# LingmaFuture/PRCV2025REID

Hardware: AMD Instinct MI355X
Metric: multimodal instances/sec (PxK, 5-modality) at 1/2/4/8 GPU; eval queries/sec (higher is better)
Workload: dtype bf16; 1 GPU; P=16,K=4 per GPU, vis/nir/sk/cp 224x224 + text (T<=77), CLIP ViT-B/16 + text tower random-init, MER-LoRA r=8, masks all-on, 400 ids, SDM+CE, fwd+bwd+grad sanitise/clip+AdamW (reference default trainable set); P=16, K=4, global_batch=64, lora_rank=8, accum_steps=1, parallelism=dp1

## Files before the change

### include/reid_hip.h

```cpp
#ifndef REID_HIP_H
#define REID_HIP_H

#include <stdint.h>

#ifdef __cplusplus
extern "C" {
#endif

typedef enum {
    REID_OK = 0,
    REID_ERR_ARG = -1,
    REID_ERR_LAUNCH = -2,
    REID_ERR_DEVICE = -3
} reid_status;

typedef enum { REID_BF16 = 0, REID_F32 = 1, REID_F16 = 2 } reid_dtype;

typedef enum {
    REID_ACT_NONE = 0,
    REID_ACT_GELU_ERF = 1,
    REID_ACT_QUICK_GELU = 2,
    REID_ACT_RELU = 3,
    REID_ACT_DGELU_ERF = 4,
    REID_ACT_DQUICK_GELU = 5,
// ... 41 lines not shown
int reid_add_layernorm_fwd(const float* x, int32_t ldx, const void* y_bf16, int32_t y_dtype, int32_t ldy, const float* row_scale, int32_t rows_per_img,
                           float* x_out, int32_t ldxo, const float* gamma, const float* beta, void* h_bf16, int32_t ldh,
                           float* mean, float* rstd, int32_t rows, int32_t cols, float eps, void* stream);
int reid_layernorm_bwd(const void* dy, int32_t dy_dtype, int32_t lddy, const float* x, int32_t ldx,
                       const int32_t* row_index, const float* gamma, const float* mean, const float* rstd,
                       const void* dres, void* dx, int32_t dx_dtype, void* dx_bf16, int32_t lddx,
                       float* dgamma, float* dbeta, int32_t rows, int32_t cols,
                       const float* bf16_row_scale, int32_t rows_per_img, int32_t* overflow, void* stream);

int reid_patch_im2col(const float* images, void* patches, int32_t n_img, int32_t H, int32_t W,
                      int32_t patch, int32_t cin, void* stream);
int reid_cls_rows(const float* cls, const float* pos0, float* x, int32_t ldx, int32_t n_img,
                  int32_t tokens, int32_t cols, void* stream);

int reid_attn_fwd(const void* qkv, int32_t ld, const uint8_t* key_mask, void* out, int32_t ldo, float* lse,
                  int32_t n_seq, int32_t S, int32_t heads, int32_t causal, int32_t q_tiles, void* stream);
int reid_attn_bwd(const void* qkv, int32_t ld, const uint8_t* key_mask, const void* out, const void* dout,
                  int32_t ldo, const float* lse, void* dqkv, int32_t lddqkv, float* delta_ws,
                  int32_t n_seq, int32_t S, int32_t heads, int32_t causal, int32_t q_tiles, void* stream);

int reid_cast_f32_bf16(const float* src, void* dst, int64_t n, void* stream);
int reid_cast_bf16_f32(const void* src, float* dst, int64_t n, void* stream);
int reid_pack_bf16_table(const float* src, void* dst_bf16, const int64_t* table, int32_t n_entries, void* stream);
int reid_lora_bwd_fused(const void* dY, int32_t lddy, const void* T, int32_t ldt, const void* BT, int32_t ldbt, void* U, int32_t ldu,
                        float* dB, int32_t lddb, const int32_t* img_mod, int32_t rows_per_img, int32_t mask_r, int32_t M, int32_t N,
                        int32_t Rp, float scale, float* u_partial, int32_t u_mode, void* stream);
int reid_lora_da_fused(const void* X, int32_t ldx, const void* U, int32_t ldu, float* dA, int32_t ldda, const int32_t* img_mod,
                       int32_t rows_per_img, int32_t mask_r, int32_t M, int32_t K, int32_t Rp, int32_t n_groups, void* stream);

int reid_merge_lora_table(const int64_t* table, int32_t n_entries, int32_t max_tiles, const float* arena, void* weff,
                          int32_t Rp, int32_t r, int32_t nmod, float scaling, void* stream);
int reid_gather_rows_f32(const float* src, int32_t lds, const int32_t* index, float* dst, int32_t ldd,
                         int32_t rows, int32_t cols, void* stream);
int reid_embed_tokens(const float* tok, const float* pos, const int64_t* ids, float* out, int32_t B, int32_t T, int32_t D,
                      int32_t vocab, void* stream);
int reid_scatter_add_rows_f32(const float* src, int32_t lds, const int32_t* index, float* out, int32_t ldo,
                              int32_t rows, int32_t cols, int32_t out_rows, void* stream);

int reid_bnneck_stats(const float* x, int32_t ldx, int32_t rows, int32_t D, float* sum, float* sqsum, void* stream);
int reid_bnneck_fwd(const float* x, int32_t ldx, const float* gamma, const float* beta, float* running_mean,
                    float* running_var, const float* sum, const float* sqsum, float count, int32_t training,
                    float* y, void* y_bf16, int32_t ldy, float* mean, float* invstd, float* rnorm,
                    int32_t rows, int32_t D, float eps, float momentum, float scale, void* stream);
int reid_bnneck_bwd_p1(const float* dy, int32_t lddy, const float* x, int32_t ldx, const float* gamma,
                       const float* beta, const float* mean, const float* invstd, const float* rnorm,
                       float* dz, float* sum_dz, float* sum_dz_xhat, int32_t rows, int32_t D, float scale,
                       void* stream);
int reid_bnneck_bwd_p2(const float* dz, const float* x, int32_t ldx, const float* gamma, const float* mean,
                       const float* invstd, const float* sum_dz, const float* sum_dz_xhat, float count,
                       int32_t training, float* dx, int32_t lddx, int32_t rows, int32_t D, void* stream);

// ... 67 lines not shown
```

### prcv2025reid_amd/_lib.py

```python
import ctypes as C
import os

import torch

_HERE = os.path.dirname(os.path.abspath(__file__))
LIB_PATHS = {'bf16': os.path.join(_HERE, 'csrc', 'libreid_hip.so'), 'f16': os.path.join(_HERE, 'csrc', 'libreid_hip_f16.so')}
if os.environ.get('REID_LIB_BF16'):
    LIB_PATHS['bf16'] = os.environ['REID_LIB_BF16']
LIB_PATH = LIB_PATHS['bf16']
T16_DTYPES = {'bf16': torch.bfloat16, 'f16': torch.float16}
_flavor = os.environ.get('REID_T16', 'bf16')


def set_flavor(name: str):
    global _flavor
    if name not in LIB_PATHS:
        raise ValueError(f'unknown 16-bit flavor {name!r}')
    _flavor = name


def flavor() -> str:
    return _flavor


# ... 23 lines not shown
                ('b_group_stride', C.c_int64)]


_P, _I, _I64, _F, _S = C.c_void_p, C.c_int32, C.c_int64, C.c_float, C.c_char_p
_GEMM = C.POINTER(GemmArgs)
SIGNATURES = {
    'reid_last_error': (_S, []),
    'reid_version': (_I, []),
    'reid_flavor': (_I, []),
    'reid_check_device': (_I, [_I]),
    'reid_set_knob': (_I, [_S, _I]),
    'reid_mer_gemm': (_I, [_GEMM, _P]),
    'reid_gemm_tn': (_I, [_P, _P, _P, _I, _I, _I, _I, _I, _I, _F, _F, _P]),
    'reid_layernorm_fwd': (_I, [_P, _I, _P, _P, _P, _P, _P, _I, _P, _P, _I, _I, _F, _P]),
    'reid_add_layernorm_fwd': (_I, [_P, _I, _P, _I, _I, _P, _I, _P, _I, _P, _P, _P, _I, _P, _P, _I, _I, _F, _P]),
    'reid_layernorm_bwd': (_I, [_P, _I, _I, _P, _I, _P, _P, _P, _P, _P, _P, _I, _P, _I, _P, _P, _I, _I, _P, _I, _P, _P]),
    'reid_patch_im2col': (_I, [_P, _P, _I, _I, _I, _I, _I, _P]),
    'reid_cls_rows': (_I, [_P, _P, _P, _I, _I, _I, _I, _P]),
    'reid_attn_fwd': (_I, [_P, _I, _P, _P, _I, _P, _I, _I, _I, _I, _I, _P]),
    'reid_attn_bwd': (_I, [_P, _I, _P, _P, _P, _I, _P, _P, _I, _P, _I, _I, _I, _I, _I, _P]),
    'reid_cast_f32_bf16': (_I, [_P, _P, _I64, _P]),
    'reid_cast_bf16_f32': (_I, [_P, _P, _I64, _P]),
    'reid_pack_bf16_table': (_I, [_P, _P, _P, _I, _P]),
    'reid_lora_bwd_fused': (_I, [_P, _I, _P, _I, _P, _I, _P, _I, _P, _I, _P, _I, _I, _I, _I, _I, _F, _P, _I, _P]),
    'reid_lora_da_fused': (_I, [_P, _I, _P, _I, _P, _I, _P, _I, _I, _I, _I, _I, _I, _P]),
    'reid_merge_lora_table': (_I, [_P, _I, _I, _P, _P, _I, _I, _I, _F, _P]),
    'reid_gather_rows_f32': (_I, [_P, _I, _P, _P, _I, _I, _I, _P]),
    'reid_embed_tokens': (_I, [_P, _P, _P, _P, _I, _I, _I, _I, _P]),
    'reid_scatter_add_rows_f32': (_I, [_P, _I, _P, _P, _I, _I, _I, _I, _P]),
    'reid_bnneck_stats': (_I, [_P, _I, _I, _I, _P, _P, _P]),
    'reid_bnneck_fwd': (_I, [_P, _I, _P, _P, _P, _P, _P, _P, _F, _I, _P, _P, _I, _P, _P, _P, _I, _I, _F, _F, _F, _P]),
    'reid_bnneck_bwd_p1': (_I, [_P, _I, _P, _I, _P, _P, _P, _P, _P, _P, _P, _P, _I, _I, _F, _P]),
    'reid_bnneck_bwd_p2': (_I, [_P, _P, _I, _P, _P, _P, _P, _P, _F, _I, _P, _I, _I, _I, _P]),
    'reid_ce_ls_fwd': (_I, [_P, _I, _P, _P, _I, _I, _F, _P, _P, _P]),
    'reid_ce_ls_bwd': (_I, [_P, _I, _P, _P, _I, _I, _F, _P, _P, _I, _P]),
    'reid_sdm_fwd': (_I, [_P, _I, _P, _I, _P, _P, _P, _P, _I, _I, _I, _I, _F, _P, _P, _P]),
    'reid_sdm_bwd': (_I, [_P, _I, _P, _I, _P, _P, _P, _P, _I, _I, _I, _I, _F, _P, _P, _P, _I, _P, _I, _P]),
    'reid_sdm_ws_floats': (_I64, [_I, _I, _I, _I]),
    'reid_topk_ws_bytes': (_I64, [_I, _I, _I]),
    'reid_topk_scan_ok': (_I, [_I, _I, _I, _I]),
    'reid_cosine_topk': (_I, [_P, _P, _P, _P, _I, _I, _I, _I, _P, _P, _P, _P, _P, _P]),
    'reid_cosine_topk_exact': (_I, [_P, _P, _I, _I, _I, _I, _P, _P, _P, _P, _P, _P]),
    'reid_cosine_topk_exact_slots': (_I, [_P, _P, _I, _I, _I, _I, _P, _P, _I, _P, _P, _P, _P, _P]),
    'reid_topk_stream_ok': (_I, [_I, _I, _I, _I]),
    'reid_topk_stream_ws_bytes': (_I64, [_I]),
    'reid_cosine_topk_stream': (_I, [_P, _P, _I, _I, _I, _I, _P, _P, _P, _P, _P, _P]),
    'reid_sgemm': (_I, [_P, _P, _P, _I, _I, _I, _I64, _I64, _I64, _I64, _I, _F, _F, _P, _I, _P]),
    'reid_eltwise_f32': (_I, [_I, _P, _P, _P, _I64, _F, _P]),
# ... 91 lines not shown
```

### prcv2025reid_amd/csrc/lora.hip

```cpp
#include "common.h"
#include <type_traits>

namespace {

constexpr int MT = 64;

__global__ __launch_bounds__(256) void merge_lora_kernel(const int64_t* __restrict__ table, const float* __restrict__ arena,
                                                         bf16_t* __restrict__ weff, int Rp, int r, int nmod, float s) {
    REID_T16_ENTER();
    const int64_t* e = table + (size_t)blockIdx.y * 8;
    const int N = (int)e[5], K = (int)e[6], G = (int)e[7];
    const int tiles_k = K / MT;
    if ((int)blockIdx.x >= (N / MT) * tiles_k) return;
    const float* __restrict__ W = (const float*)e[0];
    const float* __restrict__ A = arena + e[1];
    const float* __restrict__ B = arena + e[2];
    bf16_t* dst = weff + e[3];
    bf16_t* dstT = e[4] >= 0 ? weff + e[4] : nullptr;
    const int n0 = ((int)blockIdx.x / tiles_k) * MT, k0 = ((int)blockIdx.x % tiles_k) * MT;
    const int g = n0 / (N / G);
    const int R = nmod * r;
    __shared__ __attribute__((aligned(16))) float sW[MT][MT + 4];
    __shared__ __attribute__((aligned(16))) float sA[MT][MT + 4];
    __shared__ __attribute__((aligned(16))) float sBt[MT][MT + 4];
// ... 67 lines not shown
}

namespace fused {
constexpr int N = 768, RP = 32, R = 32;
constexpr int TP = RP * 2 + 32;
template <int NW> struct Geo {
    static constexpr int CPW = N / NW, MT = CPW / 16, KS = CPW / 32, CH = CPW / 8, XL = R * CH / 64;
    static constexpr int XP = CPW * 2 + 32;
    static constexpr int WAVE_LDS = R * XP + R * TP;
    static constexpr int LDS_BYTES = NW * WAVE_LDS + NW * R * RP * 4;
};

typedef __attribute__((ext_vector_type(4))) short s4;
typedef __attribute__((address_space(3))) s4* lds_s4_ptr;
typedef float f32x2v __attribute__((ext_vector_type(2)));

struct Params {
    const bf16_t* dY; const bf16_t* T; const bf16_t* BT; bf16_t* U; float* dB;
    const int32_t* img_mod;
    int lddy, ldt, ldbt, ldu, lddb, rows_per_img, mask_r, M, slab_rows;
    float scale;
    float* Up;
    int u_mode;
};

__device__ __forceinline__ bf16x8 tr_frag(const char* img, int pitch, int k0, int col0, int lane) {
    const int l16 = lane & 15, fq = lane >> 4;
    const int q = l16 >> 2, pp = l16 & 3;
    const char* a0 = img + (k0 + 4 * fq + q) * pitch + (col0 + 4 * pp) * 2;
    const s4 lo = __builtin_amdgcn_ds_read_tr16_b64_v4i16((lds_s4_ptr)(a0));
    const s4 hi = __builtin_amdgcn_ds_read_tr16_b64_v4i16((lds_s4_ptr)(a0 + 16 * pitch));
    return bf16x8{lo[0], lo[1], lo[2], lo[3], hi[0], hi[1], hi[2], hi[3]};
}

template <int NW>
__global__ __launch_bounds__(NW * 64, 2) void lora_bwd_fused_kernel(const Params p) {
    REID_T16_ENTER();
    using G = Geo<NW>;
    constexpr int CPW = G::CPW, MT = G::MT, KS = G::KS, CH = G::CH, XL = G::XL, XP = G::XP, WAVE_LDS = G::WAVE_LDS;
    extern __shared__ __attribute__((aligned(16))) char smem[];
    const int tid = threadIdx.x, lane = tid & 63;
    const int w = __builtin_amdgcn_readfirstlane(tid >> 6);
    const int l16 = lane & 15, fq = lane >> 4;
    char* xs = smem + w * WAVE_LDS;
    char* ts = xs + R * XP;
    float* ured = (float*)(smem + NW * WAVE_LDS);
// ... 86 lines not shown
    gload(0);
    for (int t = 0; t < steps; ++t) step(t);
#pragma unroll
    for (int i = 0; i < MT; ++i)
#pragma unroll
        for (int j = 0; j < 2; ++j)
#pragma unroll
            for (int e = 0; e < 4; ++e)
                atomicAdd(p.dB + (size_t)(col0 + i * 16 + 4 * fq + e) * p.lddb + j * 16 + l16, acc[i][j][e]);
}
}

namespace image {
constexpr int N = fused::N, RP = fused::RP, R = 32;
constexpr int ROW_BYTES = N * 2;
constexpr int IMG_BYTES = R * ROW_BYTES;
constexpr int T_BYTES = R * RP * 2;
constexpr int BUF_BYTES = IMG_BYTES + T_BYTES;
constexpr int NBUF = 3;
constexpr int USTAGE_BYTES = R * RP * 2;
constexpr int LDS_BYTES = NBUF * BUF_BYTES + USTAGE_BYTES;
typedef const __attribute__((address_space(1))) void* gptr_t;
typedef __attribute__((address_space(3))) void* lptr_t;
using fused::s4; using fused::lds_s4_ptr; using fused::Params;

typedef __attribute__((address_space(3))) char* lds_cptr;
__device__ __forceinline__ uint32_t lds_addr(const char* ptr) { return (uint32_t)(uintptr_t)(lds_cptr)(char*)ptr; }
__device__ __forceinline__ void dma16(const void* src, uint32_t lds_base) {
    const uint32_t m0v = __builtin_amdgcn_readfirstlane(lds_base);
    asm volatile("s_mov_b32 m0, %1\n\ts_nop 0\n\tglobal_load_lds_dwordx4 %0, off" ::"v"(src), "s"(m0v) : "memory");
}

__device__ __forceinline__ bf16x8 tr_frag_swz(const char* img, int col0, int lane) {
    const int l16 = lane & 15, fq = lane >> 4;
    const int q = l16 >> 2, pp = l16 & 3;
    const int col = col0 + 4 * pp;
    const int r0 = 4 * fq + q, r1 = r0 + 16;
    const char* a0 = img + r0 * ROW_BYTES + (((col >> 3) ^ (r0 & 15)) << 4) + (col & 7) * 2;
    const char* a1 = img + r1 * ROW_BYTES + (((col >> 3) ^ (r1 & 15)) << 4) + (col & 7) * 2;
    const s4 lo = __builtin_amdgcn_ds_read_tr16_b64_v4i16((lds_s4_ptr)a0);
    const s4 hi = __builtin_amdgcn_ds_read_tr16_b64_v4i16((lds_s4_ptr)a1);
    return bf16x8{lo[0], lo[1], lo[2], lo[3], hi[0], hi[1], hi[2], hi[3]};
}

__global__ __launch_bounds__(256) void u_finish_kernel(const float* __restrict__ Up, bf16_t* __restrict__ U, int ldu, const int32_t* __restrict__ img_mod,
                                                       int rows_per_img, int mask_r, float scale, int M) {
    REID_T16_ENTER();
// ... 132 lines not shown
                }
            }
            const int cbase = (w - 2) * 128;
#pragma unroll
            for (int i = 0; i < 8; ++i) acc[i] = mfma16(tr_frag_swz(xs, cbase + i * 16, lane), tf, acc[i]);
        }
        const int nb = buf == 0 ? NBUF - 1 : buf - 1;
        if (t + 2 < steps) issue(t + 2, nb);
        buf = buf + 1 == NBUF ? 0 : buf + 1;
    }
    if (w < 2) flush_pending();
    __syncthreads();
    float* fl = (float*)smem;
    if (w >= 2) {
        const int cbase = (w - 2) * 128;
#pragma unroll
        for (int i = 0; i < 8; ++i)
#pragma unroll
            for (int e = 0; e < 4; ++e) fl[(cbase + i * 16 + 4 * fq + e) * 16 + l16] = acc[i][e];
    }
    __syncthreads();
    {
        const int rr = p.mask_r, total = N * rr;
        for (int idx = tid; idx < total; idx += 512) {
            const int col = idx / rr, j = idx - col * rr;
            atomicAdd(p.dB + (size_t)col * p.lddb + mu * rr + j, fl[col * 16 + c_lo + j]);
        }
    }
}

struct DaParams {
    const bf16_t* X; const bf16_t* U; float* dA;
    const int32_t* img_mod;
    int ldx, ldu, ldda, rows_per_img, mask_r, M, Rp;
};
template <int G>
__global__ __launch_bounds__(512, 2) void lora_da_image_kernel(const DaParams p) {
    REID_T16_ENTER();
    constexpr int UB = 4096;
    constexpr int BUF = IMG_BYTES + UB;
    extern __shared__ __attribute__((aligned(16))) char smem[];
    const int tid = threadIdx.x, lane = tid & 63;
    const int w = __builtin_amdgcn_readfirstlane(tid >> 6);
    const int l16 = lane & 15, fq = lane >> 4;
    const int img = blockIdx.x, cblk = blockIdx.y;
    const int rbeg = img * p.rows_per_img;
    const int rend = min(p.M, rbeg + p.rows_per_img);
    if (rbeg >= rend) return;
    const int mu = p.img_mod[img];
    const int w0 = (mu * p.mask_r) & ~15;
    const int c_lo = mu * p.mask_r - w0, c_hi = c_lo + p.mask_r;
    const int steps = (rend - rbeg + R - 1) / R;
    const bf16_t* Xb = p.X + (size_t)cblk * N;
    const uint32_t smem_a = lds_addr(smem);
    auto issue = [&](int t, int buf) {
        const uint32_t base = smem_a + buf * BUF;
        const int r0 = rbeg + t * R;
// ... 33 lines not shown
        const char* xs = smem + buf * BUF;
        const char* us = xs + IMG_BYTES;
        const int nvalid = rend - (rbeg + t * R);
        bf16x8 uf[G];
#pragma unroll
        for (int g = 0; g < G; ++g) {
            uf[g] = fused::tr_frag(us + g * 1024, 32, 0, 0, lane);
            if (nvalid < R) {
#pragma unroll
                for (int j = 0; j < 8; ++j)
                    if (16 * (j >> 2) + 4 * fq + (j & 3) >= nvalid) uf[g][j] = 0;
            }
        }
#pragma unroll
        for (int i = 0; i < 6; ++i) {
            const bf16x8 xf = tr_frag_swz(xs, w * 96 + i * 16, lane);
#pragma unroll
            for (int g = 0; g < G; ++g) acc[g][i] = mfma16(uf[g], xf, acc[g][i]);
        }
        const int nb = buf == 0 ? NBUF - 1 : buf - 1;
        if (t + 2 < steps) issue(t + 2, nb);
        buf = buf + 1 == NBUF ? 0 : buf + 1;
    }
#pragma unroll
    for (int e = 0; e < 4; ++e) {
        const int c = 4 * fq + e;
        if (c < c_lo || c >= c_hi) continue;
#pragma unroll
        for (int g = 0; g < G; ++g)
#pragma unroll
            for (int i = 0; i < 6; ++i)
                atomicAdd(p.dA + (size_t)(g * p.Rp + w0 + c) * p.ldda + (size_t)cblk * N + w * 96 + i * 16 + l16, acc[g][i][e]);
    }
}
}

}

extern "C" int reid_lora_bwd_fused(const void* dY, int32_t lddy, const void* T, int32_t ldt, const void* BT, int32_t ldbt, void* U,
                                   int32_t ldu, float* dB, int32_t lddb, const int32_t* img_mod, int32_t rows_per_img, int32_t mask_r,
                                   int32_t M, int32_t N, int32_t Rp, float scale, float* u_partial, int32_t u_mode, void* stream) {
    REID_CHECK_ARG(u_mode >= 0 && u_mode <= 3 && (u_mode == 0 || u_partial), "reid_lora_bwd_fused: u_mode=%d needs u_partial", u_mode);
    REID_CHECK_ARG(dY && T && BT && U && dB && img_mod, "reid_lora_bwd_fused: null pointer");
    REID_CHECK_ARG(N == fused::N && Rp == fused::RP, "reid_lora_bwd_fused: N=%d Rp=%d (this kernel is built for N = 768, Rp = 32)", N, Rp);
    REID_CHECK_ARG(M > 0 && rows_per_img > 0 && mask_r > 0 && mask_r <= Rp, "reid_lora_bwd_fused: M=%d rows_per_img=%d mask_r=%d", M, rows_per_img, mask_r);
    REID_CHECK_ARG(lddy % 8 == 0 && ldt % 8 == 0 && ldbt % 8 == 0 && ldu % 2 == 0 && lddy >= N && ldt >= Rp && ldbt >= N && ldu >= Rp && lddb >= Rp,
                   "reid_lora_bwd_fused: leading dimensions");
    REID_CHECK_ARG(((uintptr_t)dY | (uintptr_t)T | (uintptr_t)BT) % 16 == 0 && (uintptr_t)U % 4 == 0, "reid_lora_bwd_fused: operand alignment");
    fused::Params p{(const bf16_t*)dY, (const bf16_t*)T, (const bf16_t*)BT, (bf16_t*)U, dB, img_mod, lddy, ldt, ldbt, ldu, lddb, rows_per_img,
                    mask_r, M, 0, scale, u_partial, u_mode};
    if (reid_knob(KNOB_LORA_IMPL) != 1 && rows_per_img >= image::R && mask_r <= 16 && 16 % mask_r == 0) {
        REID_MAX_LDS((image::lora_bwd_image_kernel), image::LDS_BYTES);
        const int n_img = (M + rows_per_img - 1) / rows_per_img;
        hipLaunchKernelGGL(image::lora_bwd_image_kernel, dim3(n_img), dim3(512), image::LDS_BYTES, (hipStream_t)stream, p);
        REID_CHECK_LAUNCH("reid_lora_bwd_fused(image)");
        if (u_mode == 1) {
            hipLaunchKernelGGL(image::u_finish_kernel, dim3((M * 16 + 255) / 256), dim3(256), 0, (hipStream_t)stream, (const float*)u_partial, (bf16_t*)U,
                               ldu, img_mod, rows_per_img, mask_r, scale, M);
            REID_CHECK_LAUNCH("reid_lora_bwd_fused(finish)");
        }
        return REID_OK;
    }
    int slabs = 64;
    p.slab_rows = ((M + slabs - 1) / slabs + fused::R - 1) / fused::R * fused::R;
    slabs = (M + p.slab_rows - 1) / p.slab_rows;
    REID_MAX_LDS((fused::lora_bwd_fused_kernel<8>), fused::Geo<8>::LDS_BYTES);
    hipLaunchKernelGGL(fused::lora_bwd_fused_kernel<8>, dim3(slabs), dim3(512), fused::Geo<8>::LDS_BYTES, (hipStream_t)stream, p);
    REID_CHECK_LAUNCH("reid_lora_bwd_fused");
    return REID_OK;
}

extern "C" int reid_lora_da_fused(const void* X, int32_t ldx, const void* U, int32_t ldu, float* dA, int32_t ldda, const int32_t* img_mod,
                                  int32_t rows_per_img, int32_t mask_r, int32_t M, int32_t K, int32_t Rp, int32_t n_groups, void* stream) {
    REID_CHECK_ARG(X && U && dA && img_mod, "reid_lora_da_fused: null pointer");
    REID_CHECK_ARG(M > 0 && K > 0 && K % 768 == 0 && Rp == 32 && (n_groups == 1 || n_groups == 3), "reid_lora_da_fused: M=%d K=%d Rp=%d groups=%d (K a multiple of 768, Rp = 32, 1 or 3 groups)", M, K, Rp, n_groups);
    REID_CHECK_ARG(rows_per_img >= image::R && mask_r > 0 && mask_r <= 16 && 16 % mask_r == 0, "reid_lora_da_fused: rows_per_img=%d (>= 32) mask_r=%d (a divisor of 16)", rows_per_img, mask_r);
    REID_CHECK_ARG(ldx % 8 == 0 && ldu % 8 == 0 && ldx >= K && ldu >= n_groups * Rp && ldda >= K, "reid_lora_da_fused: leading dimensions");
    REID_CHECK_ARG(((uintptr_t)X | (uintptr_t)U) % 16 == 0, "reid_lora_da_fused: operand alignment");
    image::DaParams p{(const bf16_t*)X, (const bf16_t*)U, dA, img_mod, ldx, ldu, ldda, rows_per_img, mask_r, M, Rp};
    const int n_img = (M + rows_per_img - 1) / rows_per_img;
    constexpr int LDS = image::NBUF * (image::IMG_BYTES + 4096);
    if (n_groups == 1) {
        REID_MAX_LDS((image::lora_da_image_kernel<1>), LDS);
        hipLaunchKernelGGL(image::lora_da_image_kernel<1>, dim3(n_img, K / 768), dim3(512), LDS, (hipStream_t)stream, p);
    } else {
        REID_MAX_LDS((image::lora_da_image_kernel<3>), LDS);
        hipLaunchKernelGGL(image::lora_da_image_kernel<3>, dim3(n_img, K / 768), dim3(512), LDS, (hipStream_t)stream, p);
    }
    REID_CHECK_LAUNCH("reid_lora_da_fused");
    return REID_OK;
}

extern "C" int reid_merge_lora_table(const int64_t* table, int32_t n_entries, int32_t max_tiles, const float* arena, void* weff,
                                     int32_t Rp, int32_t r, int32_t nmod, float scaling, void* stream) {
    REID_CHECK_ARG(table && arena && weff, "reid_merge_lora_table: null pointer");
    REID_CHECK_ARG(n_entries > 0 && n_entries <= 65535 && max_tiles > 0, "reid_merge_lora_table: n_entries=%d max_tiles=%d", n_entries, max_tiles);
    REID_CHECK_ARG(r > 0 && nmod > 0 && r <= MT && nmod * r <= Rp, "reid_merge_lora_table: r = %d must be <= %d and nmod*r = %d <= Rp = %d", r, MT, nmod * r, Rp);
    hipLaunchKernelGGL(merge_lora_kernel, dim3(max_tiles, n_entries), dim3(256), 0, (hipStream_t)stream, table, arena, (bf16_t*)weff, Rp, r, nmod,
                       scaling);
    REID_CHECK_LAUNCH("reid_merge_lora_table");
    return REID_OK;
}
```

### prcv2025reid_amd/engine.py

```python
from collections import OrderedDict
from typing import Dict, List, Optional, Tuple

import os

import torch

from . import _lib, ops

LIN = ('qkv', 'out', 'fc1', 'fc2')


def round_up(a, b):
    return (a + b - 1) // b * b


class LoraLayout:

    def __init__(self, arch):
        self.vmods = [m for m in arch['modalities'] if m != 'text']
        self.nmod = len(self.vmods)
        self.r = arch['lora_rank']
        self.Rp = round_up(self.nmod * self.r, 32)
        self.d = arch['vision_hidden_dim']; self.ff = arch['vision_mlp_dim']
        self.L = arch['vision_layers']
# ... 411 lines not shown
        dgf, dbf = ln_grads(ce + 'vision_ln_final')
        ops.layernorm_bwd(dcls, st['x_final'], P[ce + 'vision_ln_final.weight'], st['mf'], st['rf'], dx_c, dx_bf16=dxb_c,
                          bf16_row_scale=st['layers'][-1]['sm'], rows_per_img=1, dgamma=dgf, dbeta=dbf, overflow=ovf)
        U2 = torch.empty(M, Rp, **b16); U1 = torch.empty(M, Rp, **b16); Uo = torch.empty(M, Rp, **b16)
        Uq = torch.empty(M, 3 * Rp, **b16)
        du2 = [torch.empty(M, ff, **b16) for _ in range(2)]
        dqkv2 = [torch.empty(M, 3 * d, **b16) for _ in range(2)]
        dxmb2 = [torch.empty(M, d, **b16) for _ in range(2)]
        dxb2 = [dxb, torch.empty(M, d, **b16)]
        dh = torch.empty(M, d, **b16); do = torch.empty(M, d, **b16)
        delta = torch.empty(n_img, heads, S, **f32)
        dxm = torch.empty(M, d, **gx)
        weT = lambda l, nm: lay.weff(self._weff, l, nm, transposed=True)
        rg_full, rg_cls = st['rg_full'], st['rg_cls']
        main = torch.cuda.current_stream(dev)
        side = self._side_stream() if self.overlap_tn else None
        side_done = {}
        L = a['vision_layers']
        u_part = torch.empty(M, Rp, **f32)
        cls_tmp = dict(U2=torch.empty(n_img, Rp, **b16), U1=torch.empty(n_img, Rp, **b16), Uo=torch.empty(n_img, Rp, **b16),
                       du=torch.empty(n_img, ff, **b16), dh=torch.empty(n_img, d, **b16), do=torch.empty(n_img, d, **b16),
                       dxm=torch.empty(n_img, d, **gx), dxmb=torch.empty(n_img, d, **b16))

        def lora_grads(l, calls):
            def run():
                for dY, BT, U, kw, tns in calls:
                    same = tns[0][0].data_ptr() == dY.data_ptr() and tns[0][0].shape == dY.shape and tns[0][0].stride() == dY.stride()
                    if same and ops.lora_bwd_fused_ok(dY.shape[1], tns[0][1].shape[1]):
                        ops.lora_bwd_fused(dY, tns[0][1], BT, U, tns[0][2], kw['img_mod'], kw['rows_per_img'], kw['mask_r'], kw['alpha'],
                                           u_partial=u_part[:dY.shape[0]] if dY.shape[1] > 768 else None)
                        rest = tns[1:]
                    else:
                        ops.gemm(dY, BT, U, **kw)
                        rest = tns
                    for xx, yy, out in rest:
                        ng = xx.shape[1] // Rp
                        if xx.shape[1] == ng * Rp and out.shape[0] == ng * Rp and \
                                ops.lora_da_fused_ok(yy.shape[1], Rp, kw['rows_per_img'], kw['mask_r'], ng):
                            ops.lora_da_fused(yy, xx, out, kw['img_mod'], kw['rows_per_img'], kw['mask_r'], n_groups=ng)
                        else:
                            ops.gemm_tn(xx, yy, out, beta=1.0)
            if side is None:
                run()
                return
            ev = torch.cuda.Event(); ev.record(main); side.wait_event(ev)
            with torch.cuda.stream(side):
                run()

        def layer_done(l):
            if side is not None:
                ev = torch.cuda.Event(); ev.record(side); side_done[l] = ev

        def wait_side(l):
            ev = side_done.pop(l, None)
            if ev is not None:
                main.wait_event(ev)

        for l in reversed(range(L)):
            s = st['layers'][l]
            lp = f'{ce}vision_layers.{l}.'
            b = l & 1
            c = bool(s.get('cls'))
            if c:
                Mr, rg = n_img, rg_cls
                mkr = dict(img_mod=st['img_mod'], mask_r=r, mask_period=Rp, rows_per_img=1, alpha=self.scaling)
                gy, gyb = dx_c, dxb_c
                U2r, U1r, Uor, dur, dhr, dor, dxmr, dxmbr = (cls_tmp[k_] for k_ in ('U2', 'U1', 'Uo', 'du', 'dh', 'do', 'dxm', 'dxmb'))
                rpi = 1
            else:
                Mr, mkr, gy, gyb, rg = M, mk, dx, dxb2[b], rg_full
                U2r, U1r, Uor, dur, dhr, dor, dxmr, dxmbr, rpi = U2, U1, Uo, du2[b], dh, do, dxm, dxmb2[b], S
            dqkv = dqkv2[b]
            lora_grads(l, [(gyb, pk(l, 'fc2', 'BT'), U2r, mkr, [(gyb, s['T2'], gB(l, 'fc2')), (U2r, s['g'], gA(l, 'fc2'))])])
            ops.gemm(gyb, weT(l, 'fc2'), dur, act='mul_aux', aux=s['u'], row_groups=rg)
# ... 260 lines not shown
```

### prcv2025reid_amd/ops.py

```python
import ctypes as C
from typing import Optional

import torch

from . import _lib as L
from ._lib import BF16, F32, GemmArgs, check, lib, ptr, stream_ptr

ACT = {'none': L.ACT_NONE, 'gelu': L.ACT_GELU, 'quick_gelu': L.ACT_QUICK_GELU, 'relu': L.ACT_RELU,
       'dgelu': L.ACT_DGELU, 'dquick_gelu': L.ACT_DQUICK_GELU, 'drelu': L.ACT_DRELU,
       'mul_aux': L.ACT_MUL_AUX, 'gelu_dsave': L.ACT_GELU_DSAVE}


_gemm_profile = None
def gemm_profile_begin():
    global _gemm_profile
    _gemm_profile = []


def gemm_profile_end():
    global _gemm_profile
    p, _gemm_profile = _gemm_profile, None
    return p


# ... 116 lines not shown
    n, _, H, W = images.shape
    check(lib().reid_patch_im2col(ptr(images), ptr(patches), n, H, W, patch, cin, stream_ptr()))


def cls_rows(cls, pos0, x, n_img, tokens):
    check(lib().reid_cls_rows(ptr(cls), ptr(pos0), ptr(x), x.stride(0), n_img, tokens, x.shape[1], stream_ptr()))


def attn_fwd(qkv, out, lse, n_seq, S, heads, causal=False, key_mask=None, q_tiles=0):
    check(lib().reid_attn_fwd(ptr(qkv), qkv.stride(0), ptr(key_mask), ptr(out), out.stride(0), ptr(lse), n_seq, S, heads,
                              int(causal), int(q_tiles), stream_ptr()))


def attn_bwd(qkv, out, dout, lse, dqkv, delta_ws, n_seq, S, heads, causal=False, key_mask=None, q_tiles=0):
    check(lib().reid_attn_bwd(ptr(qkv), qkv.stride(0), ptr(key_mask), ptr(out), ptr(dout), out.stride(0), ptr(lse),
                              ptr(dqkv), dqkv.stride(0), ptr(delta_ws), n_seq, S, heads, int(causal), int(q_tiles), stream_ptr()))


def cast_f32_bf16(src, dst):
    check(lib().reid_cast_f32_bf16(ptr(src), ptr(dst), src.numel(), stream_ptr()))
    return dst


def lora_bwd_fused(dY, T, BT, U, dB, img_mod, rows_per_img, mask_r, scale, u_partial=None):
    N = dY.shape[1]
    nb = N // 768
    if nb > 1 and u_partial is None:
        raise ValueError('lora_bwd_fused: a cotangent wider than 768 columns needs u_partial')
    for q in range(nb):
        mode = 0 if nb == 1 else ((1 if q > 0 else 0) | (2 if q + 1 < nb else 0))
        dYq, BTq, dBq = dY[:, q * 768:(q + 1) * 768], BT[:, q * 768:(q + 1) * 768], dB[q * 768:(q + 1) * 768]
        check(lib().reid_lora_bwd_fused(ptr(dYq), dYq.stride(0), ptr(T), T.stride(0), ptr(BTq), BTq.stride(0), ptr(U), U.stride(0),
                                        ptr(dBq), dBq.stride(0), ptr(img_mod), rows_per_img, mask_r, dY.shape[0], 768, T.shape[1],
                                        scale, ptr(u_partial), mode, stream_ptr()))


def lora_da_fused(X, U, dA, img_mod, rows_per_img, mask_r, n_groups=1):
    check(lib().reid_lora_da_fused(ptr(X), X.stride(0), ptr(U), U.stride(0), ptr(dA), dA.stride(0), ptr(img_mod), rows_per_img, mask_r,
                                   X.shape[0], X.shape[1], U.shape[1] // n_groups, n_groups, stream_ptr()))


def lora_da_fused_ok(K, Rp, rows_per_img, mask_r, n_groups):
    return K % 768 == 0 and Rp == 32 and rows_per_img >= 32 and mask_r <= 16 and 16 % mask_r == 0 and n_groups in (1, 3)


def lora_bwd_fused_ok(N, Rp):
    return N % 768 == 0 and N // 768 in (1, 2, 3, 4) and Rp == 32


def merge_lora_table(table, n_entries, max_tiles, arena, weff, Rp, r, nmod, scaling):
    check(lib().reid_merge_lora_table(ptr(table), n_entries, max_tiles, ptr(arena), ptr(weff), Rp, r, nmod, scaling, stream_ptr()))


def to_bf16(src: torch.Tensor) -> torch.Tensor:
    src = src.contiguous()
    dst = torch.empty(src.shape, dtype=L.t16(), device=src.device)
    if src.numel():
        cast_f32_bf16(src, dst)
    return dst


def pack_bf16_table(src_arena, dst_arena, table, n_entries):
# ... 149 lines not shown
```

Baseline: 2131 instances/s.

## Replace LoRA gradient atomics with per-image partials and batched deferred reduction

The fused LoRA backward kernels (dB and dA) used to atomically add per-image contributions into the gradient buffers. They now write per-image partials into a per-stream workspace. A new batched reduce kernel sums those partials by modality mask, and it runs once per layer for up to 16 entries. This targets atomic contention and nondeterminism, at the cost of extra workspace memory, extra memory traffic, and an additional reduce launch per layer.

Result: no change. 2129 instances/s, median of 3 (-0.1%).

```diff
diff --git a/include/reid_hip.h b/include/reid_hip.h
--- a/include/reid_hip.h
+++ b/include/reid_hip.h
@@ -87,11 +87,14 @@
 int reid_cast_f32_bf16(const float* src, void* dst, int64_t n, void* stream);
 int reid_cast_bf16_f32(const void* src, float* dst, int64_t n, void* stream);
 int reid_pack_bf16_table(const float* src, void* dst_bf16, const int64_t* table, int32_t n_entries, void* stream);
-int reid_lora_bwd_fused(const void* dY, int32_t lddy, const void* T, int32_t ldt, const void* BT, int32_t ldbt, void* U, int32_t ldu,
-                        float* dB, int32_t lddb, const int32_t* img_mod, int32_t rows_per_img, int32_t mask_r, int32_t M, int32_t N,
-                        int32_t Rp, float scale, float* u_partial, int32_t u_mode, void* stream);
-int reid_lora_da_fused(const void* X, int32_t ldx, const void* U, int32_t ldu, float* dA, int32_t ldda, const int32_t* img_mod,
-                       int32_t rows_per_img, int32_t mask_r, int32_t M, int32_t K, int32_t Rp, int32_t n_groups, void* stream);
+int reid_lora_bwd_fused_ws(const void* dY, int32_t lddy, const void* T, int32_t ldt, const void* BT, int32_t ldbt, void* U, int32_t ldu,
+                           float* dB, int32_t lddb, const int32_t* img_mod, int32_t rows_per_img, int32_t mask_r, int32_t M, int32_t N,
+                           int32_t Rp, float scale, float* u_partial, int32_t u_mode, float* workspace, int64_t workspace_bytes,
+                           int32_t defer, void* stream);
+int reid_lora_da_fused_ws(const void* X, int32_t ldx, const void* U, int32_t ldu, float* dA, int32_t ldda, const int32_t* img_mod,
+                          int32_t rows_per_img, int32_t mask_r, int32_t M, int32_t K, int32_t Rp, int32_t n_groups, float* workspace,
+                          int64_t workspace_bytes, int32_t defer, void* stream);
+int reid_lora_reduce_partials(const int64_t* entries, int32_t n_entries, void* stream);
 
 int reid_merge_lora_table(const int64_t* table, int32_t n_entries, int32_t max_tiles, const float* arena, void* weff,
                           int32_t Rp, int32_t r, int32_t nmod, float scaling, void* stream);
diff --git a/prcv2025reid_amd/_lib.py b/prcv2025reid_amd/_lib.py
--- a/prcv2025reid_amd/_lib.py
+++ b/prcv2025reid_amd/_lib.py
@@ -69,8 +69,9 @@
     'reid_cast_f32_bf16': (_I, [_P, _P, _I64, _P]),
     'reid_cast_bf16_f32': (_I, [_P, _P, _I64, _P]),
     'reid_pack_bf16_table': (_I, [_P, _P, _P, _I, _P]),
-    'reid_lora_bwd_fused': (_I, [_P, _I, _P, _I, _P, _I, _P, _I, _P, _I, _P, _I, _I, _I, _I, _I, _F, _P, _I, _P]),
-    'reid_lora_da_fused': (_I, [_P, _I, _P, _I, _P, _I, _P, _I, _I, _I, _I, _I, _I, _P]),
+    'reid_lora_bwd_fused_ws': (_I, [_P, _I, _P, _I, _P, _I, _P, _I, _P, _I, _P, _I, _I, _I, _I, _I, _F, _P, _I, _P, _I64, _I, _P]),
+    'reid_lora_da_fused_ws': (_I, [_P, _I, _P, _I, _P, _I, _P, _I, _I, _I, _I, _I, _I, _P, _I64, _I, _P]),
+    'reid_lora_reduce_partials': (_I, [_P, _I, _P]),
     'reid_merge_lora_table': (_I, [_P, _I, _I, _P, _P, _I, _I, _I, _F, _P]),
     'reid_gather_rows_f32': (_I, [_P, _I, _P, _P, _I, _I, _I, _P]),
     'reid_embed_tokens': (_I, [_P, _P, _P, _P, _I, _I, _I, _I, _P]),
diff --git a/prcv2025reid_amd/csrc/lora.hip b/prcv2025reid_amd/csrc/lora.hip
--- a/prcv2025reid_amd/csrc/lora.hip
+++ b/prcv2025reid_amd/csrc/lora.hip
@@ -113,6 +113,7 @@
     float scale;
     float* Up;
     int u_mode;
+    float* dBp;
 };
 
 __device__ __forceinline__ bf16x8 tr_frag(const char* img, int pitch, int k0, int col0, int lane) {
@@ -245,7 +246,7 @@
 constexpr int LDS_BYTES = NBUF * BUF_BYTES + USTAGE_BYTES;
 typedef const __attribute__((address_space(1))) void* gptr_t;
 typedef __attribute__((address_space(3))) void* lptr_t;
-using fused::s4; using fused::lds_s4_ptr; using fused::Params;
+using fused::s4; using fused::lds_s4_ptr; using fused::Params; using fused::f32x2v;
 
 typedef __attribute__((address_space(3))) char* lds_cptr;
 __device__ __forceinline__ uint32_t lds_addr(const char* ptr) { return (uint32_t)(uintptr_t)(lds_cptr)(char*)ptr; }
@@ -424,17 +425,18 @@
     __syncthreads();
     {
         const int rr = p.mask_r, total = N * rr;
+        float* part = p.dBp + (size_t)img * total;
         for (int idx = tid; idx < total; idx += 512) {
             const int col = idx / rr, j = idx - col * rr;
-            atomicAdd(p.dB + (size_t)col * p.lddb + mu * rr + j, fl[col * 16 + c_lo + j]);
+            part[idx] = fl[col * 16 + c_lo + j];
         }
     }
 }
 
 struct DaParams {
-    const bf16_t* X; const bf16_t* U; float* dA;
+    const bf16_t* X; const bf16_t* U; float* dAp;
     const int32_t* img_mod;
-    int ldx, ldu, ldda, rows_per_img, mask_r, M, Rp;
+    int ldx, ldu, rows_per_img, mask_r, M, Rp;
 };
 template <int G>
 __global__ __launch_bounds__(512, 2) void lora_da_image_kernel(const DaParams p) {
@@ -514,6 +516,8 @@
         if (t + 2 < steps) issue(t + 2, nb);
         buf = buf + 1 == NBUF ? 0 : buf + 1;
     }
+    const int rr = p.mask_r;
+    float* part = p.dAp + ((size_t)img * gridDim.y + cblk) * G * rr * N;
 #pragma unroll
     for (int e = 0; e < 4; ++e) {
         const int c = 4 * fq + e;
@@ -521,35 +525,135 @@
 #pragma unroll
         for (int g = 0; g < G; ++g)
 #pragma unroll
-            for (int i = 0; i < 6; ++i)
-                atomicAdd(p.dA + (size_t)(g * p.Rp + w0 + c) * p.ldda + (size_t)cblk * N + w * 96 + i * 16 + l16, acc[g][i][e]);
-    }
-}
-}
-
-}
-
-extern "C" int reid_lora_bwd_fused(const void* dY, int32_t lddy, const void* T, int32_t ldt, const void* BT, int32_t ldbt, void* U,
-                                   int32_t ldu, float* dB, int32_t lddb, const int32_t* img_mod, int32_t rows_per_img, int32_t mask_r,
-                                   int32_t M, int32_t N, int32_t Rp, float scale, float* u_partial, int32_t u_mode, void* stream) {
-    REID_CHECK_ARG(u_mode >= 0 && u_mode <= 3 && (u_mode == 0 || u_partial), "reid_lora_bwd_fused: u_mode=%d needs u_partial", u_mode);
-    REID_CHECK_ARG(dY && T && BT && U && dB && img_mod, "reid_lora_bwd_fused: null pointer");
-    REID_CHECK_ARG(N == fused::N && Rp == fused::RP, "reid_lora_bwd_fused: N=%d Rp=%d (this kernel is built for N = 768, Rp = 32)", N, Rp);
-    REID_CHECK_ARG(M > 0 && rows_per_img > 0 && mask_r > 0 && mask_r <= Rp, "reid_lora_bwd_fused: M=%d rows_per_img=%d mask_r=%d", M, rows_per_img, mask_r);
+            for (int i = 0; i < 6; ++i) part[(size_t)(g * rr + c - c_lo) * N + w * 96 + i * 16 + l16] = acc[g][i][e];
+    }
+}
+
+enum { RED_DB = 0, RED_DA = 1 };
+struct RedEntry {
+    const float* part; float* dst; const int32_t* img_mod;
+    int n_img, Q, r, ld, G, mode;
+};
+constexpr int RED_MAX = 16, RED_Q = 128, RED_U = 16;
+struct RedBatch { RedEntry e[RED_MAX]; };
+
+__device__ __forceinline__ size_t red_dst(const RedEntry& p, int q, int mu) {
+    if (p.mode == RED_DB) {
+        const int col = q / p.r, j = q - col * p.r;
+        return (size_t)col * p.ld + mu * p.r + j;
+    }
+    const int k = q % N, a = q / N;
+    const int j = a % p.r, cg = a / p.r, g = cg % p.G, cblk = cg / p.G;
+    return (size_t)(g * RP + mu * p.r + j) * p.ld + (size_t)cblk * N + k;
+}
+
+template <int NMU, int NW>
+__global__ __launch_bounds__(NW * 64) void lora_partial_reduce_kernel(const RedBatch b) {
+    REID_T16_ENTER();
+    __shared__ __attribute__((aligned(16))) float red[NW][RED_Q];
+    __shared__ unsigned presw[NW];
+    const RedEntry p = b.e[blockIdx.y];
+    if ((int)blockIdx.x * RED_Q >= p.Q) return;
+    const int tid = threadIdx.x, lane = tid & 63;
+    const int w = __builtin_amdgcn_readfirstlane(tid >> 6);
+    const int q0 = blockIdx.x * RED_Q + 2 * lane;
+    float dv[NMU];
+    if (tid < RED_Q) {
+#pragma unroll
+        for (int k = 0; k < NMU; ++k) dv[k] = k * p.r < RP ? p.dst[red_dst(p, blockIdx.x * RED_Q + tid, k)] : 0.f;
+    }
+    const int i0 = (int)((int64_t)p.n_img * w / NW), i1 = (int)((int64_t)p.n_img * (w + 1) / NW);
+    f32x2v acc[NMU];
+#pragma unroll
+    for (int k = 0; k < NMU; ++k) acc[k] = f32x2v{0.f, 0.f};
+    unsigned pres = 0u;
+    for (int i = i0; i < i1; i += RED_U) {
+        const int mv = lane < RED_U && i + lane < i1 ? p.img_mod[i + lane] : -1;
+        f32x2v v[RED_U];
+#pragma unroll
+        for (int u = 0; u < RED_U; ++u) {
+            const int ii = min(i + u, i1 - 1);
+            v[u] = *(const f32x2v*)(p.part + (size_t)ii * p.Q + q0);
+        }
+#pragma unroll
+        for (int u = 0; u < RED_U; ++u) {
+            const int mu = __builtin_amdgcn_readlane(mv, u);
+            if (mu >= 0 && mu < NMU) pres |= 1u << mu;
+#pragma unroll
+            for (int k = 0; k < NMU; ++k)
+                if (mu == k) acc[k] += v[u];
+        }
+    }
+    if (lane == 0) presw[w] = pres;
+    __syncthreads();
+    unsigned all = 0u;
+#pragma unroll
+    for (int ww = 0; ww < NW; ++ww) all |= presw[ww];
+#pragma unroll
+    for (int k = 0; k < NMU; ++k) {
+        if (!((all >> k) & 1u)) continue;
+        *(f32x2v*)&red[w][2 * lane] = acc[k];
+        __syncthreads();
+        if (tid < RED_Q) {
+            float s = red[0][tid];
+#pragma unroll
+            for (int ww = 1; ww < NW; ++ww) s += red[ww][tid];
+            p.dst[red_dst(p, blockIdx.x * RED_Q + tid, k)] = dv[k] + s;
+        }
+        __syncthreads();
+    }
+}
+
+int launch_partial_reduce(const RedBatch& b, int n, hipStream_t stream) {
+    int rmin = 16, qmax = 0;
+    for (int i = 0; i < n; ++i) { rmin = min(rmin, b.e[i].r); qmax = max(qmax, b.e[i].Q); }
+    const dim3 grid(qmax / RED_Q, n);
+    const int nmu = RP / rmin;
+    if (nmu <= 4) hipLaunchKernelGGL((lora_partial_reduce_kernel<4, 16>), grid, dim3(16 * 64), 0, stream, b);
+    else if (nmu <= 8) hipLaunchKernelGGL((lora_partial_reduce_kernel<8, 16>), grid, dim3(16 * 64), 0, stream, b);
+    else if (nmu <= 16) hipLaunchKernelGGL((lora_partial_reduce_kernel<16, 8>), grid, dim3(8 * 64), 0, stream, b);
+    else hipLaunchKernelGGL((lora_partial_reduce_kernel<32, 8>), grid, dim3(8 * 64), 0, stream, b);
+    return 0;
+}
+}
+
+}
+
+extern "C" int reid_lora_bwd_fused_ws(const void* dY, int32_t lddy, const void* T, int32_t ldt, const void* BT, int32_t ldbt, void* U,
+                                      int32_t ldu, float* dB, int32_t lddb, const int32_t* img_mod, int32_t rows_per_img, int32_t mask_r,
+                                      int32_t M, int32_t N, int32_t Rp, float scale, float* u_partial, int32_t u_mode, float* workspace,
+                                      int64_t workspace_bytes, int32_t defer, void* stream) {
+    REID_CHECK_ARG(u_mode >= 0 && u_mode <= 3 && (u_mode == 0 || u_partial), "reid_lora_bwd_fused_ws: u_mode=%d needs u_partial", u_mode);
+    REID_CHECK_ARG(dY && T && BT && U && dB && img_mod, "reid_lora_bwd_fused_ws: null pointer");
+    REID_CHECK_ARG(N == fused::N && Rp == fused::RP, "reid_lora_bwd_fused_ws: N=%d Rp=%d (this kernel is built for N = 768, Rp = 32)", N, Rp);
+    REID_CHECK_ARG(M > 0 && rows_per_img > 0 && mask_r > 0 && mask_r <= Rp, "reid_lora_bwd_fused_ws: M=%d rows_per_img=%d mask_r=%d", M, rows_per_img, mask_r);
     REID_CHECK_ARG(lddy % 8 == 0 && ldt % 8 == 0 && ldbt % 8 == 0 && ldu % 2 == 0 && lddy >= N && ldt >= Rp && ldbt >= N && ldu >= Rp && lddb >= Rp,
-                   "reid_lora_bwd_fused: leading dimensions");
-    REID_CHECK_ARG(((uintptr_t)dY | (uintptr_t)T | (uintptr_t)BT) % 16 == 0 && (uintptr_t)U % 4 == 0, "reid_lora_bwd_fused: operand alignment");
+                   "reid_lora_bwd_fused_ws: leading dimensions");
+    REID_CHECK_ARG(((uintptr_t)dY | (uintptr_t)T | (uintptr_t)BT) % 16 == 0 && (uintptr_t)U % 4 == 0, "reid_lora_bwd_fused_ws: operand alignment");
+    const bool image_shape = rows_per_img >= image::R && mask_r <= 16 && 16 % mask_r == 0;
+    const int n_img = (M + rows_per_img - 1) / rows_per_img;
+    const int64_t need = (int64_t)n_img * N * mask_r * (int64_t)sizeof(float);
+    REID_CHECK_ARG(!defer || image_shape, "reid_lora_bwd_fused_ws: defer needs the one-image-per-workgroup shape (rows_per_img >= 32, mask_r a divisor of 16)");
     fused::Params p{(const bf16_t*)dY, (const bf16_t*)T, (const bf16_t*)BT, (bf16_t*)U, dB, img_mod, lddy, ldt, ldbt, ldu, lddb, rows_per_img,
-                    mask_r, M, 0, scale, u_partial, u_mode};
-    if (reid_knob(KNOB_LORA_IMPL) != 1 && rows_per_img >= image::R && mask_r <= 16 && 16 % mask_r == 0) {
+                    mask_r, M, 0, scale, u_partial, u_mode, workspace};
+    if (image_shape) {
+        REID_CHECK_ARG(workspace && workspace_bytes >= need && (uintptr_t)workspace % 16 == 0,
+                       "reid_lora_bwd_fused_ws: workspace of %lld bytes (16-byte aligned) needed, %lld given", (long long)need, (long long)workspace_bytes);
+    }
+    if (image_shape && reid_knob(KNOB_LORA_IMPL) != 1) {
         REID_MAX_LDS((image::lora_bwd_image_kernel), image::LDS_BYTES);
-        const int n_img = (M + rows_per_img - 1) / rows_per_img;
         hipLaunchKernelGGL(image::lora_bwd_image_kernel, dim3(n_img), dim3(512), image::LDS_BYTES, (hipStream_t)stream, p);
-        REID_CHECK_LAUNCH("reid_lora_bwd_fused(image)");
+        REID_CHECK_LAUNCH("reid_lora_bwd_fused_ws(image)");
+        if (!defer) {
+            image::RedBatch b{};
+            b.e[0] = image::RedEntry{workspace, dB, img_mod, n_img, N * mask_r, mask_r, lddb, 1, image::RED_DB};
+            image::launch_partial_reduce(b, 1, (hipStream_t)stream);
+            REID_CHECK_LAUNCH("reid_lora_bwd_fused_ws(reduce)");
+        }
         if (u_mode == 1) {
             hipLaunchKernelGGL(image::u_finish_kernel, dim3((M * 16 + 255) / 256), dim3(256), 0, (hipStream_t)stream, (const float*)u_partial, (bf16_t*)U,
                                ldu, img_mod, rows_per_img, mask_r, scale, M);
-            REID_CHECK_LAUNCH("reid_lora_bwd_fused(finish)");
+            REID_CHECK_LAUNCH("reid_lora_bwd_fused_ws(finish)");
         }
         return REID_OK;
     }
@@ -558,19 +662,26 @@
     slabs = (M + p.slab_rows - 1) / p.slab_rows;
     REID_MAX_LDS((fused::lora_bwd_fused_kernel<8>), fused::Geo<8>::LDS_BYTES);
     hipLaunchKernelGGL(fused::lora_bwd_fused_kernel<8>, dim3(slabs), dim3(512), fused::Geo<8>::LDS_BYTES, (hipStream_t)stream, p);
-    REID_CHECK_LAUNCH("reid_lora_bwd_fused");
+    REID_CHECK_LAUNCH("reid_lora_bwd_fused_ws");
+    if (defer) {
+        REID_CHECK_HIP(hipMemsetAsync(workspace, 0, (size_t)need, (hipStream_t)stream), "reid_lora_bwd_fused_ws(zero partials)");
+    }
     return REID_OK;
 }
 
-extern "C" int reid_lora_da_fused(const void* X, int32_t ldx, const void* U, int32_t ldu, float* dA, int32_t ldda, const int32_t* img_mod,
-                                  int32_t rows_per_img, int32_t mask_r, int32_t M, int32_t K, int32_t Rp, int32_t n_groups, void* stream) {
-    REID_CHECK_ARG(X && U && dA && img_mod, "reid_lora_da_fused: null pointer");
-    REID_CHECK_ARG(M > 0 && K > 0 && K % 768 == 0 && Rp == 32 && (n_groups == 1 || n_groups == 3), "reid_lora_da_fused: M=%d K=%d Rp=%d groups=%d (K a multiple of 768, Rp = 32, 1 or 3 groups)", M, K, Rp, n_groups);
-    REID_CHECK_ARG(rows_per_img >= image::R && mask_r > 0 && mask_r <= 16 && 16 % mask_r == 0, "reid_lora_da_fused: rows_per_img=%d (>= 32) mask_r=%d (a divisor of 16)", rows_per_img, mask_r);
-    REID_CHECK_ARG(ldx % 8 == 0 && ldu % 8 == 0 && ldx >= K && ldu >= n_groups * Rp && ldda >= K, "reid_lora_da_fused: leading dimensions");
-    REID_CHECK_ARG(((uintptr_t)X | (uintptr_t)U) % 16 == 0, "reid_lora_da_fused: operand alignment");
-    image::DaParams p{(const bf16_t*)X, (const bf16_t*)U, dA, img_mod, ldx, ldu, ldda, rows_per_img, mask_r, M, Rp};
+extern "C" int reid_lora_da_fused_ws(const void* X, int32_t ldx, const void* U, int32_t ldu, float* dA, int32_t ldda, const int32_t* img_mod,
+                                     int32_t rows_per_img, int32_t mask_r, int32_t M, int32_t K, int32_t Rp, int32_t n_groups, float* workspace,
+                                     int64_t workspace_bytes, int32_t defer, void* stream) {
+    REID_CHECK_ARG(X && U && dA && img_mod, "reid_lora_da_fused_ws: null pointer");
+    REID_CHECK_ARG(M > 0 && K > 0 && K % 768 == 0 && Rp == 32 && (n_groups == 1 || n_groups == 3), "reid_lora_da_fused_ws: M=%d K=%d Rp=%d groups=%d (K a multiple of 768, Rp = 32, 1 or 3 groups)", M, K, Rp, n_groups);
+    REID_CHECK_ARG(rows_per_img >= image::R && mask_r > 0 && mask_r <= 16 && 16 % mask_r == 0, "reid_lora_da_fused_ws: rows_per_img=%d (>= 32) mask_r=%d (a divisor of 16)", rows_per_img, mask_r);
+    REID_CHECK_ARG(ldx % 8 == 0 && ldu % 8 == 0 && ldx >= K && ldu >= n_groups * Rp && ldda >= K, "reid_lora_da_fused_ws: leading dimensions");
+    REID_CHECK_ARG(((uintptr_t)X | (uintptr_t)U) % 16 == 0, "reid_lora_da_fused_ws: operand alignment");
     const int n_img = (M + rows_per_img - 1) / rows_per_img;
+    const int64_t need = (int64_t)n_img * K * n_groups * mask_r * (int64_t)sizeof(float);
+    REID_CHECK_ARG(workspace && workspace_bytes >= need && (uintptr_t)workspace % 16 == 0,
+                   "reid_lora_da_fused_ws: workspace of %lld bytes (16-byte aligned) needed, %lld given", (long long)need, (long long)workspace_bytes);
+    image::DaParams p{(const bf16_t*)X, (const bf16_t*)U, workspace, img_mod, ldx, ldu, rows_per_img, mask_r, M, Rp};
     constexpr int LDS = image::NBUF * (image::IMG_BYTES + 4096);
     if (n_groups == 1) {
         REID_MAX_LDS((image::lora_da_image_kernel<1>), LDS);
@@ -579,7 +690,30 @@
         REID_MAX_LDS((image::lora_da_image_kernel<3>), LDS);
         hipLaunchKernelGGL(image::lora_da_image_kernel<3>, dim3(n_img, K / 768), dim3(512), LDS, (hipStream_t)stream, p);
     }
-    REID_CHECK_LAUNCH("reid_lora_da_fused");
+    REID_CHECK_LAUNCH("reid_lora_da_fused_ws");
+    if (!defer) {
+        image::RedBatch b{};
+        b.e[0] = image::RedEntry{workspace, dA, img_mod, n_img, K * n_groups * mask_r, mask_r, ldda, n_groups, image::RED_DA};
+        image::launch_partial_reduce(b, 1, (hipStream_t)stream);
+        REID_CHECK_LAUNCH("reid_lora_da_fused_ws(reduce)");
+    }
+    return REID_OK;
+}
+
+extern "C" int reid_lora_reduce_partials(const int64_t* entries, int32_t n_entries, void* stream) {
+    REID_CHECK_ARG(entries && n_entries > 0 && n_entries <= image::RED_MAX, "reid_lora_reduce_partials: n_entries=%d (1..%d)", n_entries, image::RED_MAX);
+    image::RedBatch b{};
+    for (int i = 0; i < n_entries; ++i) {
+        const int64_t* e = entries + (size_t)i * 9;
+        const int kind = (int)e[0], n_img = (int)e[5], r = (int)e[6], K = (int)e[7], G = (int)e[8];
+        REID_CHECK_ARG((kind == 0 || kind == 1) && e[1] && e[2] && e[4] && e[1] % 16 == 0 && n_img > 0 && r > 0 && r <= 16 && 16 % r == 0 &&
+                       (kind == 0 ? (K == 768 && G == 1 && e[3] >= 32) : (K > 0 && K % 768 == 0 && (G == 1 || G == 3) && e[3] >= K)),
+                       "reid_lora_reduce_partials: entry %d {kind %d, n_img %d, mask_r %d, K %d, groups %d, ld %lld}", i, kind, n_img, r, K, G, (long long)e[3]);
+        b.e[i] = image::RedEntry{(const float*)e[1], (float*)e[2], (const int32_t*)e[4], n_img, K * G * r, r, (int)e[3], G,
+                                 kind == 0 ? image::RED_DB : image::RED_DA};
+    }
+    image::launch_partial_reduce(b, n_entries, (hipStream_t)stream);
+    REID_CHECK_LAUNCH("reid_lora_reduce_partials");
     return REID_OK;
 }
 
diff --git a/prcv2025reid_amd/engine.py b/prcv2025reid_amd/engine.py
--- a/prcv2025reid_amd/engine.py
+++ b/prcv2025reid_amd/engine.py
@@ -457,13 +457,15 @@
                        du=torch.empty(n_img, ff, **b16), dh=torch.empty(n_img, d, **b16), do=torch.empty(n_img, d, **b16),
                        dxm=torch.empty(n_img, d, **gx), dxmb=torch.empty(n_img, d, **b16))
 
+        parts = ops.LoraPartials()
+
         def lora_grads(l, calls):
             def run():
                 for dY, BT, U, kw, tns in calls:
                     same = tns[0][0].data_ptr() == dY.data_ptr() and tns[0][0].shape == dY.shape and tns[0][0].stride() == dY.stride()
                     if same and ops.lora_bwd_fused_ok(dY.shape[1], tns[0][1].shape[1]):
                         ops.lora_bwd_fused(dY, tns[0][1], BT, U, tns[0][2], kw['img_mod'], kw['rows_per_img'], kw['mask_r'], kw['alpha'],
-                                           u_partial=u_part[:dY.shape[0]] if dY.shape[1] > 768 else None)
+                                           u_partial=u_part[:dY.shape[0]] if dY.shape[1] > 768 else None, partials=parts)
                         rest = tns[1:]
                     else:
                         ops.gemm(dY, BT, U, **kw)
@@ -472,7 +474,7 @@
                         ng = xx.shape[1] // Rp
                         if xx.shape[1] == ng * Rp and out.shape[0] == ng * Rp and \
                                 ops.lora_da_fused_ok(yy.shape[1], Rp, kw['rows_per_img'], kw['mask_r'], ng):
-                            ops.lora_da_fused(yy, xx, out, kw['img_mod'], kw['rows_per_img'], kw['mask_r'], n_groups=ng)
+                            ops.lora_da_fused(yy, xx, out, kw['img_mod'], kw['rows_per_img'], kw['mask_r'], n_groups=ng, partials=parts)
                         else:
                             ops.gemm_tn(xx, yy, out, beta=1.0)
             if side is None:
@@ -483,8 +485,12 @@
                 run()
 
         def layer_done(l):
-            if side is not None:
-                ev = torch.cuda.Event(); ev.record(side); side_done[l] = ev
+            if side is None:
+                parts.flush()
+                return
+            with torch.cuda.stream(side):
+                parts.flush()
+            ev = torch.cuda.Event(); ev.record(side); side_done[l] = ev
 
         def wait_side(l):
             ev = side_done.pop(l, None)
diff --git a/prcv2025reid_amd/ops.py b/prcv2025reid_amd/ops.py
--- a/prcv2025reid_amd/ops.py
+++ b/prcv2025reid_amd/ops.py
@@ -162,22 +162,81 @@
     return dst
 
 
-def lora_bwd_fused(dY, T, BT, U, dB, img_mod, rows_per_img, mask_r, scale, u_partial=None):
+_lora_ws = {}
+
+
+def _lora_workspace(nbytes, device):
+    stream = torch.cuda.current_stream(device)
+    key = (stream.device_index, stream.cuda_stream)
+    ws = _lora_ws.get(key)
+    if ws is None or ws.numel() * 4 < nbytes:
+        ws = torch.empty((max(nbytes, 0 if ws is None else 2 * ws.numel() * 4) + 3) // 4, dtype=torch.float32, device=device)
+        _lora_ws[key] = ws
+    return ws
+
+
+class LoraPartials:
+
+    def __init__(self):
+        self.entries, self.keep, self.off, self.ws = [], [], 0, None
+
+    def take(self, nbytes, device):
+        ws = _lora_workspace(self.off + nbytes, device)
+        if ws is not self.ws:
+            if self.ws is not None:
+                self.keep.append(self.ws)
+            self.ws, self.off = ws, 0
+        p = ws.data_ptr() + self.off
+        self.off += (nbytes + 255) // 256 * 256
+        return p
+
+    def add(self, kind, ws_ptr, dst, img_mod, n_img, mask_r, K, n_groups):
+        self.entries.append((kind, ws_ptr, dst.data_ptr(), dst.stride(0), img_mod.data_ptr(), n_img, mask_r, K, n_groups))
+
+    def flush(self):
+        for i in range(0, len(self.entries), 16):
+            chunk = self.entries[i:i + 16]
+            arr = (C.c_int64 * (9 * len(chunk)))(*[v for e in chunk for v in e])
+            check(lib().reid_lora_reduce_partials(arr, len(chunk), stream_ptr()))
+        self.entries, self.keep, self.off = [], [], 0
+
+
+def _lora_image_shape(rows_per_img, mask_r):
+    return rows_per_img >= 32 and 0 < mask_r <= 16 and 16 % mask_r == 0
+
+
+def lora_bwd_fused(dY, T, BT, U, dB, img_mod, rows_per_img, mask_r, scale, u_partial=None, partials=None):
     N = dY.shape[1]
     nb = N // 768
     if nb > 1 and u_partial is None:
         raise ValueError('lora_bwd_fused: a cotangent wider than 768 columns needs u_partial')
+    image = _lora_image_shape(rows_per_img, mask_r)
+    batch = partials if partials is not None or not image else LoraPartials()
+    n_img = (dY.shape[0] + rows_per_img - 1) // rows_per_img
+    ws_bytes = n_img * 768 * mask_r * 4
     for q in range(nb):
         mode = 0 if nb == 1 else ((1 if q > 0 else 0) | (2 if q + 1 < nb else 0))
         dYq, BTq, dBq = dY[:, q * 768:(q + 1) * 768], BT[:, q * 768:(q + 1) * 768], dB[q * 768:(q + 1) * 768]
-        check(lib().reid_lora_bwd_fused(ptr(dYq), dYq.stride(0), ptr(T), T.stride(0), ptr(BTq), BTq.stride(0), ptr(U), U.stride(0),
-                                        ptr(dBq), dBq.stride(0), ptr(img_mod), rows_per_img, mask_r, dY.shape[0], 768, T.shape[1],
-                                        scale, ptr(u_partial), mode, stream_ptr()))
-
-
-def lora_da_fused(X, U, dA, img_mod, rows_per_img, mask_r, n_groups=1):
-    check(lib().reid_lora_da_fused(ptr(X), X.stride(0), ptr(U), U.stride(0), ptr(dA), dA.stride(0), ptr(img_mod), rows_per_img, mask_r,
-                                   X.shape[0], X.shape[1], U.shape[1] // n_groups, n_groups, stream_ptr()))
+        ws = batch.take(ws_bytes, dY.device) if image else None
+        check(lib().reid_lora_bwd_fused_ws(ptr(dYq), dYq.stride(0), ptr(T), T.stride(0), ptr(BTq), BTq.stride(0), ptr(U), U.stride(0),
+                                           ptr(dBq), dBq.stride(0), ptr(img_mod), rows_per_img, mask_r, dY.shape[0], 768, T.shape[1],
+                                           scale, ptr(u_partial), mode, ws, ws_bytes if image else 0, int(image), stream_ptr()))
+        if image:
+            batch.add(0, ws, dBq, img_mod, n_img, mask_r, 768, 1)
+    if image and partials is None:
+        batch.flush()
+
+
+def lora_da_fused(X, U, dA, img_mod, rows_per_img, mask_r, n_groups=1, partials=None):
+    batch = partials if partials is not None else LoraPartials()
+    n_img = (X.shape[0] + rows_per_img - 1) // rows_per_img
+    ws_bytes = n_img * X.shape[1] * n_groups * mask_r * 4
+    ws = batch.take(ws_bytes, X.device)
+    check(lib().reid_lora_da_fused_ws(ptr(X), X.stride(0), ptr(U), U.stride(0), ptr(dA), dA.stride(0), ptr(img_mod), rows_per_img, mask_r,
+                                      X.shape[0], X.shape[1], U.shape[1] // n_groups, n_groups, ws, ws_bytes, 1, stream_ptr()))
+    batch.add(1, ws, dA, img_mod, n_img, mask_r, X.shape[1], n_groups)
+    if partials is None:
+        batch.flush()
 
 
 def lora_da_fused_ok(K, Rp, rows_per_img, mask_r, n_groups):
```
